# eduardburlacu/DiTSep

Measured on AMD Instinct MI355X. Metric: separated utterances/sec @ N=30, 2-spk 4 s mixtures, higher is better.
Workload: dtype fp16 (fp16 MFMA operands, fp32 accumulate)

## Files before the change

ditsep_amd/csrc/engine.hip:

```cpp
#include <math.h>
#include <stdarg.h>
#include <stdio.h>
#include <stdlib.h>
#include <string.h>

#include <algorithm>
#include <map>
#include <numeric>
#include <set>
#include <stdexcept>
#include <string>
#include <vector>

#include "../../include/ditsep_hip.h"
#include "igemm.h"
#include "kernels.h"

namespace {

struct Err : std::runtime_error {
  int code;
  Err(int c, const std::string& m) : std::runtime_error(m), code(c) {}
};

// ... 955 lines not shown
    op16_t* lnout = fp8 ? reinterpret_cast<op16_t*>(A8) : Ap;
    const char* skx = getenv("DSN_SKINNY_MAX");
    const int skinny_max = skx ? std::min(atoi(skx), 128) : 80;
    const bool skinny = P == 1 && !fp8 && M <= skinny_max && D % 256 == 0;
    const int skinny_ks = 8;
    const bool use_panel = D % 64 == 0;
    int fold_rows = 0;
    if ((fold_ln || fold_ln8) && use_panel && !skinny) {
      for (int rounds = 1; rounds <= 4 && !fold_rows; ++rounds) {
        const int np = 256 * rounds / std::max(1, cdiv(D, 128));
        if (np >= 1 && cdiv(M, np) <= 80) fold_rows = cdiv(M, np);
      }
    }
    op16_t* Xp = (fold_rows && !fp8) ? wsbuf<op16_t>("dit_Xp", M * D) : nullptr;
    unsigned char* X8 = (fold_rows && fp8) ? wsbuf<unsigned char>("dit_X8", M * D) : nullptr;
    unsigned char* SX8 = (fold_rows && fp8) ? wsbuf<unsigned char>("dit_SX8", M * D / 32) : nullptr;
    float* ST = fold_rows ? wsbuf<float>("dit_ST", M * (D / 64) * 2) : nullptr;
    const int rot = 32;
    const bool new_rope = !ws.count("rope_cos_" + std::to_string(S));
    float* rc = wsbuf<float>("rope_cos_" + std::to_string(S), (long)S * rot);
    float* rs = wsbuf<float>("rope_sin_" + std::to_string(S), (long)S * rot);
    if (new_rope) launch_rope_tables(rc, rs, S, rot, st);

    launch_pack_tokens(xt, io, mix, Dl, B, T, nullptr, Up, Mt * din, PL, st);
    {
      Tag tg(this, "dit.project_in");
      GemmDesc d = base_desc(Up, Mt * din, pin, B, T, T);
      d.out_f32 = X;
      d.out_bstride = (long)S * D;
      d.out_off = D;
      d.out_limit = (long)S * D;
      run(d, st);
    }
    {
      const float* te = time_cache.find(t, B);
      if (!te) {
        float* tmp = wsbuf<float>("dit_te1", (long)B * D);
        Tag tg(this, "dit.time_embed");
        dit_time_embed(t, B, tmp, st);
        te = tmp;
      }
      launch_copy_rows(te, X, B, D, (long)S * D, st);
    }
    const bool short_panel = use_panel && P == 1;
    auto panel_rows_for = [&](int wg_per_panel, int max_rows = 272) {
      for (int rounds = 1;; ++rounds) {
        const int np = std::max(1, 256 * rounds / std::max(1, wg_per_panel));
        const int rows = (cdiv(M, np) + 7) / 8 * 8;
        if (rows <= max_rows) return rows;
      }
    };
    const int qkv_panel = short_panel ? 256 : 0;
    int qa_ipp = 0;
    if (P == 1 && !skinny && D == H * 64 && S <= qkv_attention_max_rows()) {
      int ipp = std::min(B, std::max(1, 144 / S));
      while (ipp > 1 && cdiv(B, ipp) * H < 256) --ipp;
      if (cdiv(B, ipp) * H >= 128) qa_ipp = ipp;
      const char* force = getenv("DSN_QA_IPP");
      if (force && atoi(force) >= 1 && atoi(force) * S <= qkv_attention_max_rows()) qa_ipp = atoi(force);
    }
    op16_t* AOp = qa_ipp ? wsbuf<op16_t>("dit_AOp", M * D) : nullptr;
    float* slabs = nullptr;
    int pend_n = 0;
    const float* pend_bias = nullptr;
    const long slab_stride = M * D;
// ... 111 lines not shown
          d.out_fp8 = H8;
          d.out_fp8_scale = SH8;
        } else {
          d.out_planes = FF;
        }
        d.out_ps = M * 4 * D;
        d.out_bstride = M * 4L * D;
        d.out_row_elems = 4 * D;
        d.out_limit = d.out_bstride;
        d.m_fast = 1;
        if (use_panel) {
          const int np = cdiv(M, 272);
          d.panel_rows = short_panel ? panel_rows_for(cdiv(4 * D * 2, 256)) : (cdiv(M, np) + 7) / 8 * 8;
        }
        if (fp8) d.panel_rows = panel_rows_for(cdiv(4 * D * 2, 256));
        layer_gemm(d, 256, use_panel);
      }
      {
        Tag tg(this, "dit.ff_out");
        GemmDesc d = layer_desc(FF, H8, SH8, L.ff2, L.ff2_8);
        stream_gemm(d, 256, 4, fp8 ? 208 : 272);
      }
    }
    prof_launch("dit.residual_norm", (double)M * D * (8.0 + 4.0 * pend_n + 2.0 * P), st, [&] {
      launch_residual_norm(X, slabs, pend_n, slab_stride, pend_bias, nullptr, nullptr, Ap, M * D, PL, (int)M, D, 1e-5f,
                           0, st);
    });
    {
      Tag tg(this, "dit.project_out");
      GemmDesc d = base_desc(Ap, M * D, pout, B, T, S);
      d.in_pad = -1;
      d.in_bstride = (long)S * D;
      d.out_f32 = SC;
      if (use_panel && P == 1 && d.N <= 128 && d.M >= 1024) {
        d.panel_rows = 64;
        run(d, st, 128);
      } else {
        run(d, st);
      }
    }
    return SC;
  }

#include "engine_ncsnpp.inc"

  float* score_tokens(const float* xt, const float* t, const float* mix, int B, int T, hipStream_t st,
                      const int* lens = nullptr) {
    if (!finalized) fail(DSN_ESTATE, "weights not finalized");
    if (cfg.score_kind == DSN_SCORE_DIT) return dit_forward(xt, t, mix, B, T, st, lens);
    if (lens) fail(DSN_EINVAL, "ragged batches need the DiT score network");
    if (cfg.score_kind == DSN_SCORE_NCSNPP) {
      Tag tg(this, "ncsnpp.conv");
      return ncsnpp_forward(xt, t, mix, B, T, st);
    }
    fail(DSN_ESTATE, "no score network configured (score_kind=%d)", cfg.score_kind);
  }

  struct Sched {
    std::vector<float> t, std, step, gain, G, g;
// ... 1823 lines not shown
        q.M = (int)M;
        q.D = t->D;
        q.H = t->H;
        q.S = t->S;
        q.ipp = t->ipp;
        q.q_scale = 0.125f;
        const hipError_t e = qkv_attention_launch(q, PL, st, lens);
        if (e != hipSuccess)
          fail(DSN_EHIP, "test_kernel qkv_attention: refused or failed: %s (D=%d H=%d S=%d ipp=%d planes=%d)",
               hipGetErrorString(e), t->D, t->H, t->S, t->ipp, P);
        break;
      }
      case DSN_TK_RESIDUAL_NORM: {
        if (!t->x || t->rows < 1 || t->D < 4 || t->D % 4 != 0 || t->D > 4096)
          fail(DSN_EINVAL, "test_kernel residual_norm: needs x, rows >= 1, D %% 4 == 0, D <= 4096 (D=%d)", t->D);
        if (t->nslab < 0 || t->nslab > 8 || (t->nslab > 0 && !t->slabs))
          fail(DSN_EINVAL, "test_kernel residual_norm: nslab %d outside [0, 8] or slabs missing", t->nslab);
        if (t->do_norm && !t->gamma) fail(DSN_EINVAL, "test_kernel residual_norm: do_norm needs gamma");
        if (!!t->out_fp8 != !!t->out_fp8_scale || (!t->out_fp8 && !oplanes))
          fail(DSN_EINVAL, "test_kernel residual_norm: needs out_planes, or out_fp8 with out_fp8_scale");
        if (t->out_fp8 && t->D % 32 != 0) fail(DSN_EINVAL, "test_kernel residual_norm: fp8 output needs D %% 32 == 0");
        launch_residual_norm(t->x, t->slabs, t->nslab, t->slab_stride, t->bias, t->gamma, t->beta,
                             t->out_fp8 ? reinterpret_cast<op16_t*>(t->out_fp8) : oplanes, t->out_ps, PL, t->rows, t->D,
                             t->eps, t->do_norm, st, t->out_fp8_scale);
        break;
      }
      case DSN_TK_GN_STATS:
      case DSN_TK_GN_APPLY: {
        if (!t->x || t->B < 1 || t->HW < 1 || t->C % 4 != 0 || !gn_groups_fit(t->C, t->C) || t->C > 1024 ||
            t->rstride < t->C || t->rstride % 4 != 0)
          fail(DSN_EINVAL, "test_kernel group norm: unsupported view (C=%d rstride=%d HW=%d)", t->C, t->rstride, t->HW);
        if (t->kind == DSN_TK_GN_STATS) {
          if (!t->out_f32) fail(DSN_EINVAL, "test_kernel gn_stats: out_f32 (the statistics) missing");
          launch_gn_stats(t->x, t->bstride, t->rstride, t->C, t->B, t->HW, t->out_f32, st);
        } else {
          if (!t->stats || !t->gamma || !t->beta || (!t->out_f32 && !oplanes))
            fail(DSN_EINVAL, "test_kernel gn_apply: stats, gamma, beta and an output are required");
          launch_gn_apply(t->x, t->bstride, t->rstride, t->C, t->B, t->HW, t->stats, t->gamma, t->beta, t->eps, t->silu,
                          t->out_f32, oplanes, t->out_ps, PL, st);
        }
        break;
      }
      case DSN_TK_FIR2D: {
        if (!t->x || t->B < 1 || t->C < 4 || t->C % 4 != 0 || t->rstride < t->C || t->rstride % 4 != 0 || t->img_h < 1 ||
            t->img_w < 1 || (!t->up && ((t->img_h | t->img_w) & 1)) || (!t->out_f32 && !oplanes))
          fail(DSN_EINVAL, "test_kernel fir2d: unsupported view (C=%d rstride=%d %d x %d up=%d)", t->C, t->rstride,
               t->img_h, t->img_w, t->up);
// ... 215 lines not shown
```

ditsep_amd/csrc/igemm.hip:

```cpp
#include "igemm.h"

#ifndef DSN_SETPRIO
#define DSN_SETPRIO 0
#endif

namespace {

constexpr int BM = 128, BN = 128, BK = 32;
constexpr int TILE_ELEMS = 128 * BK;

__device__ __forceinline__ int swz(int row, int chunk) { return chunk ^ ((-(row >> 2)) & 3); }

enum { EPI_STATS = 1, EPI_LNFOLD = 2, EPI_FP8OUT = 4 };
enum { LEAN_NO_DIT = 1, LEAN_NO_NCSN = 2, LEAN_SEEDED = 4 };

template <int NT, int MT>
__device__ __forceinline__ void seed_acc(const GemmDesc& d, f32x4 (&acc)[NT][MT], int mw0, int m_end, int nw0, int lane) {
  const int nq = (lane >> 4) * 4;
#pragma unroll
  for (int tm = 0; tm < MT; ++tm) {
    const int m = mw0 + tm * 16 + (lane & 15);
    const bool mok = m < m_end;
    const int b = mok ? m / d.rows_per_b : 0;
    const int j = mok ? m - b * d.rows_per_b : 0;
// ... 1839 lines not shown
  if (d.panel_wm == 2 && d.cfg_bk == 32 && d.Cin % 32 != 0) return hipErrorInvalidValue;
  if (d.swiglu && (d.N % 32 != 0)) return hipErrorInvalidValue;
  if (d.ksplit > 1 && (!d.out_f32 || d.swiglu)) return hipErrorInvalidValue;
  if (d.img_w > 0) return hipErrorInvalidValue;
  if (d.stat_out && (d.N % 64 != 0 || d.stat_np != d.N / 64 || d.swiglu || d.ksplit > 1)) return hipErrorInvalidValue;
  if (d.ln_stats && (!d.swiglu || !d.ln_colsum || d.ln_np <= 0 || d.taps != 1 || planes != 1)) return hipErrorInvalidValue;
  const op16_t* zp = dsn_zero_page();
  if (!zp) return hipErrorOutOfMemory;
  const int epi = (d.stat_out ? EPI_STATS : 0) | (d.ln_stats ? EPI_LNFOLD : 0);
#define PCFGE(MT_, P_, W_, NS_, BK_, E_)                                                             \
  if (planes == P_ && bn == W_ * 64 && epi == E_)                                                     \
    return f16 ? launch_panel_t<P_, 1, W_, NS_, BK_, MT_, E_>(d, zp, stream)                          \
               : launch_panel_t<P_, 0, W_, NS_, BK_, MT_, E_>(d, zp, stream);
#define PCFGS(MT_, P_, W_, NS_, BK_) PCFGE(MT_, P_, W_, NS_, BK_, 0)
#define PCFG2(MT_, NS_, BK_, E_)                                                                                \
  if (planes == 1 && bn == 256 && epi == E_ && d.panel_rows <= MT_ * 16 && (d.cfg_nst == 0 || d.cfg_nst == NS_) && \
      (d.cfg_bk == 0 || d.cfg_bk == BK_))                                                                       \
    return f16 ? launch_panel_t<1, 1, 4, NS_, BK_, MT_, E_, 2>(d, zp, stream)                                   \
               : launch_panel_t<1, 0, 4, NS_, BK_, MT_, E_, 2>(d, zp, stream);
  if (d.panel_wm == 2) {
    PCFG2(9, 3, 64, 0) PCFG2(17, 2, 64, 0) PCFG2(17, 4, 32, 0) PCFG2(17, 2, 64, EPI_LNFOLD) PCFG2(17, 4, 32, EPI_LNFOLD)
  }
#undef PCFG2
  if (d.panel_rows <= 5 * 16) {
    PCFGE(5, 1, 2, 4, 64, EPI_STATS) PCFGS(5, 1, 2, 4, 64)
  }
  if (d.panel_rows <= 7 * 16) {
    PCFGS(7, 1, 4, 3, 64) PCFGE(7, 1, 4, 3, 64, EPI_LNFOLD)
  }
  if (d.panel_rows <= 9 * 16) {
    PCFGS(9, 1, 4, 3, 64) PCFGS(9, 1, 2, 3, 64) PCFGS(9, 2, 4, 2, 32) PCFGS(9, 2, 2, 2, 32)
    PCFGE(9, 1, 4, 3, 64, EPI_LNFOLD)
  }
  if (d.panel_rows <= 13 * 16) {
    PCFGS(13, 1, 4, 2, 64) PCFGS(13, 1, 2, 2, 64) PCFGE(13, 1, 4, 2, 64, EPI_LNFOLD)
  }
  PCFGS(17, 1, 4, 2, 64) PCFGS(17, 1, 2, 2, 64) PCFGS(17, 2, 4, 2, 32) PCFGS(17, 2, 2, 2, 32)
  PCFGE(17, 1, 4, 2, 64, EPI_LNFOLD)
#undef PCFGS
#undef PCFGE
  return hipErrorInvalidValue;
}
```

ditsep_amd/csrc/kernels.h:

```cpp
#pragma once
#include "common.h"

void launch_pack_tokens(const float* src0, int C0, const float* src1, int C1, int B, int T,
                        float* dst_f32, op16_t* dst_planes, long ps, int planes, hipStream_t s);
void launch_copy_rows(const float* src, float* dst, int rows, int width, long dst_stride, hipStream_t s);
void launch_unpack_tokens(const float* src, float* dst, int B, int C, int T, hipStream_t s);
void launch_to_planes(const float* src, op16_t* dst, long ps, int planes, long n, hipStream_t s);

void launch_pc_prior(const float* mean, int mean_full, const float* z, float* x, float stdT, int B, int n, int D,
                     int T, hipStream_t s);
void launch_pc_corrector(float* x, float* x_mean , const float* score_tok, const float* z, float step,
                         float noise_gain, const float* norms, float snr, int B, int n, int D, int T, hipStream_t s);
void launch_pc_item_norms(const float* a, long per_item, int B, float* out, hipStream_t s);
void launch_pc_predictor(float* x, float* x_mean, const float* y, const float* score_tok, const float* z,
                         float theta, float dt, float G, float g, int em, int B, int n, int D, int T, hipStream_t s);

void launch_sigma_mix(const float* y, float* smix, int B, int L, int avg_len, hipStream_t s);
void launch_mix_prior(const float* y, const float* z, float* x, const float* smix, float s1, float s2, int B, int n, int D,
                      int T, hipStream_t s);
void launch_mix_corrector(float* x, float* x_mean, const float* score_tok, const float* z, const float* smix, float sq1,
                          float sq2, float snr, int B, int n, int D, int T, hipStream_t s);
void launch_mix_predictor(float* x, float* x_mean, const float* score_tok, const float* z, const float* smix,
                          float lambda, float dt, float g, float sqdt, int em, int B, int n, int D, int T, hipStream_t s);
void launch_sb_update(float* x, const float* est_tok, const float* third, float w_prev, float w_est, float w3,
                      int third_is_y, int B, int n, int D, int T, hipStream_t s);
void launch_repeat_sources(const float* y, float* x, int B, int n, int D, int T, hipStream_t s);
void launch_zero_tail(float* x, const int* lens, int B, int n, int D, int T, hipStream_t s);

void launch_residual_norm(float* x, const float* slabs, int nslab, long slab_stride, const float* bias,
                          const float* gamma, const float* beta, op16_t* out, long ps, int planes, int rows, int D,
                          float eps, int do_norm, hipStream_t s, unsigned char* out_fp8_scale = nullptr);
void launch_timestep_features(const float* t, const float* w, int B, int half, op16_t* out, long ps,
                              int planes, hipStream_t s);
hipError_t launch_attention_mfma(const op16_t* qkv, long ps, op16_t* out, long out_ps, int pl, int B, int S, int H,
                                 int dh, hipStream_t s, unsigned char* out_fp8_scale = nullptr,
                                 const int* lens = nullptr);
void launch_rope_tables(float* cos_t, float* sin_t, int S, int rot, hipStream_t s);

void launch_conv_out1(const op16_t* a, long ps, int planes, const float* w, float* out, int S, int L, int C,
                      int ktaps, int apply_tanh, hipStream_t s);
void launch_conv_in1(const float* wav, const float* w, const float* bias, int S, int L, int Cout, int ktaps,
                     float* out_f32, op16_t* out_planes, long ps, int planes, int act, const float* act_a,
                     const float* act_b, hipStream_t s);
void launch_vae_sample(const float* enc_tok, const float* noise, float* y, int S, int D, int T, hipStream_t s);

void launch_randn(float* out, long n, unsigned long long seed, unsigned long long offset, hipStream_t s);

enum { PACK_LINEAR = 0, PACK_LINEAR_SWIGLU = 1, PACK_CONV = 2, PACK_CONVT = 3, PACK_CONV2D = 4, PACK_NIN = 5 };
void launch_wn_scale(const float* v, const float* g, float* scale, int R, long inner, hipStream_t s);
void launch_pack_weight(const float* src, const float* scale, op16_t* dst, long ps, int planes, int mode,
                        int N, int K, int Cin, int Cout, int kw, int stride, hipStream_t s,
                        const float* colscale = nullptr);
void launch_packed_row_sum(const op16_t* w, long ps, int planes, int N, int K, float* out, hipStream_t s);
void launch_bias_plus_wbeta(const float* W, const float* beta, const float* bias, int N, int K, float* out,
// ... 121 lines not shown
```

ditsep_amd/csrc/kernels.hip:

```cpp
#include "kernels.h"

namespace {

constexpr int TPB = 256;
inline int grid_for(long n, int per_block = TPB, int cap = 256 * 16) {
  long g = (n + per_block - 1) / per_block;
  return (int)(g < 1 ? 1 : (g > cap ? cap : g));
}

__device__ __forceinline__ void store_planes(op16_t* dst, long ps, int planes, long i, float v) {
  op16_t h, l;
  dsn_split(v, h, l, PL_F16(planes));
  dst[i] = h;
  if (PL_COUNT(planes) == 2) dst[ps + i] = l;
}

__global__ void pack_tokens_kernel(const float* __restrict__ s0, int C0, const float* __restrict__ s1, int C1,
                                   int B, int T, float* __restrict__ df, op16_t* __restrict__ dp, long ps,
                                   int planes) {
  const int C = C0 + C1;
  const long n = (long)B * T * C;
  for (long i = blockIdx.x * (long)blockDim.x + threadIdx.x; i < n; i += (long)gridDim.x * blockDim.x) {
    const int c = (int)(i % C);
    const long bt = i / C;
    const int t = (int)(bt % T);
    const int b = (int)(bt / T);
    const float v = c < C0 ? s0[((long)b * C0 + c) * T + t] : s1[((long)b * C1 + (c - C0)) * T + t];
    if (df) df[i] = v;
    if (dp) store_planes(dp, ps, planes, i, v);
  }
}

__global__ void copy_rows_kernel(const float* __restrict__ src, float* __restrict__ dst, int rows, int width4,
                                 long dst_stride) {
  const long n = (long)rows * width4;
  for (long i = blockIdx.x * (long)blockDim.x + threadIdx.x; i < n; i += (long)gridDim.x * blockDim.x) {
    const long r = i / width4;
    const int c = (int)(i - r * width4);
    reinterpret_cast<f32x4*>(dst + r * dst_stride)[c] = reinterpret_cast<const f32x4*>(src + r * (long)width4 * 4)[c];
  }
}

__global__ void unpack_tokens_kernel(const float* __restrict__ src, float* __restrict__ dst, int B, int C, int T) {
  const long n = (long)B * C * T;
  for (long i = blockIdx.x * (long)blockDim.x + threadIdx.x; i < n; i += (long)gridDim.x * blockDim.x) {
    const int t = (int)(i % T);
    const long bc = i / T;
    const int c = (int)(bc % C);
    const int b = (int)(bc / C);
    dst[i] = src[((long)b * T + t) * C + c];
  }
}

__global__ void to_planes_kernel(const float* __restrict__ src, op16_t* __restrict__ dst, long ps, int planes,
                                 long n4) {
  for (long i = blockIdx.x * (long)blockDim.x + threadIdx.x; i < n4; i += (long)gridDim.x * blockDim.x) {
    const f32x4 v = reinterpret_cast<const f32x4*>(src)[i];
    op16x4 hi, lo;
#pragma unroll
    for (int r = 0; r < 4; ++r) {
      op16_t h, l;
      dsn_split(v[r], h, l, PL_F16(planes));
// ... 199 lines not shown
    const float th = third ? third[third_is_y ? ix.yi : i] : 0.f;
    x[i] = w_prev * x[i] + w_est * est[ix.si] + w3 * th;
  }
}
__global__ void repeat_sources_kernel(const float* __restrict__ y, float* __restrict__ x, int n, int D, int T, long total) {
  for (long i = blockIdx.x * (long)blockDim.x + threadIdx.x; i < total; i += (long)gridDim.x * blockDim.x)
    x[i] = y[pc_index(i, n, D, T).yi];
}

__global__ void zero_tail_kernel(float* __restrict__ x, const int* __restrict__ lens, int rows, int T, long total) {
  for (long i = blockIdx.x * (long)blockDim.x + threadIdx.x; i < total; i += (long)gridDim.x * blockDim.x) {
    const int t = (int)(i % T);
    const int b = (int)(i / ((long)rows * T));
    if (t >= lens[b] - 1) x[i] = 0.f;
  }
}

template <int MAXV, int NS, bool BATCH = false>
__global__ __launch_bounds__(TPB) void residual_norm_kernel(float* __restrict__ x, const float* __restrict__ slabs,
                                                            int nslab, long slab_stride, const float* __restrict__ bias,
                                                            const float* __restrict__ gamma,
                                                            const float* __restrict__ beta, op16_t* __restrict__ out,
                                                            long ps, int planes, int rows, int D, float eps, int do_norm,
                                                            unsigned char* __restrict__ o8s) {
  const int lane = threadIdx.x & 63;
  const int wpb = blockDim.x >> 6;
  const int nv = D >> 2;
  for (int row = blockIdx.x * wpb + (threadIdx.x >> 6); row < rows; row += gridDim.x * wpb) {
    const long rbase = (long)row * D;
    f32x4 v[MAXV];
    f32x4 gq[BATCH ? MAXV : 1], bq[BATCH ? MAXV : 1];
    float s = 0.f;
    if constexpr (BATCH) {
      f32x4 bv[MAXV];
      f32x4 part[NS > 0 ? NS : 1][MAXV];
#pragma unroll
      for (int k = 0; k < MAXV; ++k) {
        const int i = min(lane + k * 64, nv - 1);
        v[k] = reinterpret_cast<const f32x4*>(x + rbase)[i];
        bv[k] = (NS > 0 && bias) ? reinterpret_cast<const f32x4*>(bias)[i] : f32x4{0.f, 0.f, 0.f, 0.f};
#pragma unroll
        for (int z = 0; z < NS; ++z) part[z][k] = reinterpret_cast<const f32x4*>(slabs + z * slab_stride + rbase)[i];
      }
#pragma unroll
      for (int k = 0; k < MAXV; ++k) {
        const int i = lane + k * 64;
        if (do_norm) {
          gq[k] = reinterpret_cast<const f32x4*>(gamma)[min(i, nv - 1)];
          bq[k] = beta ? reinterpret_cast<const f32x4*>(beta)[min(i, nv - 1)] : f32x4{0.f, 0.f, 0.f, 0.f};
        }
        v[k] += bv[k];
#pragma unroll
        for (int z = 0; z < NS; ++z) v[k] += part[z][k];
        if (i < nv) {
          if (NS > 0) reinterpret_cast<f32x4*>(x + rbase)[i] = v[k];
          s += (v[k][0] + v[k][1]) + (v[k][2] + v[k][3]);
        }
      }
    } else {
#pragma unroll
      for (int k = 0; k < MAXV; ++k) {
        const int i = lane + k * 64;
        if (i < nv) {
          f32x4 a = reinterpret_cast<const f32x4*>(x + rbase)[i];
          if (NS > 0) {
            f32x4 part[NS > 0 ? NS : 1];
#pragma unroll
            for (int z = 0; z < NS; ++z) part[z] = reinterpret_cast<const f32x4*>(slabs + z * slab_stride + rbase)[i];
            if (bias) a += reinterpret_cast<const f32x4*>(bias)[i];
#pragma unroll
            for (int z = 0; z < NS; ++z) a += part[z];
            reinterpret_cast<f32x4*>(x + rbase)[i] = a;
          }
          v[k] = a;
          s += (a[0] + a[1]) + (a[2] + a[3]);
        }
      }
    }
    float mean = 0.f, rstd = 1.f;
    if (do_norm) {
      mean = wave_sum(s) / D;
      float q = 0.f;
#pragma unroll
      for (int k = 0; k < MAXV; ++k) {
        const int i = lane + k * 64;
        if (i < nv) {
#pragma unroll
          for (int r = 0; r < 4; ++r) {
            const float dlt = v[k][r] - mean;
            q += dlt * dlt;
          }
        }
      }
      rstd = rsqrtf(wave_sum(q) / D + eps);
    }
// ... 25 lines not shown
        }
        op16x4 hi, lo;
#pragma unroll
        for (int r = 0; r < 4; ++r) {
          op16_t h, l;
          dsn_split(o[r], h, l, PL_F16(planes));
          hi[r] = h;
          lo[r] = l;
        }
        const long oi = (rbase >> 2) + i;
        reinterpret_cast<op16x4*>(out)[oi] = hi;
        if (PL_COUNT(planes) == 2) reinterpret_cast<op16x4*>(out + ps)[oi] = lo;
      }
    }
  }
}

template <int NS>
__global__ __launch_bounds__(TPB) void residual_norm_row_kernel(float* __restrict__ x, const float* __restrict__ slabs,
                                                                long slab_stride, const float* __restrict__ bias,
                                                                const float* __restrict__ gamma,
                                                                const float* __restrict__ beta, op16_t* __restrict__ out,
                                                                long ps, int planes, int D, float eps, int do_norm,
                                                                unsigned char* __restrict__ o8s) {
  __shared__ float red[2][TPB / 64];
  const int i = threadIdx.x, lane = i & 63, wave = i >> 6;
  const long rbase = (long)blockIdx.x * D;
  f32x4 a = reinterpret_cast<const f32x4*>(x + rbase)[i];
  f32x4 part[NS > 0 ? NS : 1];
#pragma unroll
  for (int z = 0; z < NS; ++z) part[z] = reinterpret_cast<const f32x4*>(slabs + z * slab_stride + rbase)[i];
  f32x4 g = {1.f, 1.f, 1.f, 1.f}, be = {0.f, 0.f, 0.f, 0.f};
  if (do_norm) {
    g = reinterpret_cast<const f32x4*>(gamma)[i];
    if (beta) be = reinterpret_cast<const f32x4*>(beta)[i];
  }
  if (NS > 0) {
    if (bias) a += reinterpret_cast<const f32x4*>(bias)[i];
#pragma unroll
    for (int z = 0; z < NS; ++z) a += part[z];
    reinterpret_cast<f32x4*>(x + rbase)[i] = a;
  }
  f32x4 o = a;
  if (do_norm) {
    const float s = wave_sum((a[0] + a[1]) + (a[2] + a[3]));
    if (lane == 0) red[0][wave] = s;
    __syncthreads();
    float tot = 0.f;
#pragma unroll
    for (int w = 0; w < TPB / 64; ++w) tot += red[0][w];
    const float mean = tot / D;
    float q = 0.f;
#pragma unroll
    for (int r = 0; r < 4; ++r) {
      const float dlt = a[r] - mean;
      q += dlt * dlt;
    }
    q = wave_sum(q);
    if (lane == 0) red[1][wave] = q;
    __syncthreads();
    float qt = 0.f;
#pragma unroll
    for (int w = 0; w < TPB / 64; ++w) qt += red[1][w];
    const float rstd = rsqrtf(qt / D + eps);
// ... 436 lines not shown
  s = wave_sum(s);
  if (lane == 0) out[row] = s + (bias ? bias[row] : 0.f);
}

__global__ void pack_bias_swiglu_kernel(const float* __restrict__ src, float* __restrict__ dst, int N) {
  const int F = N / 2;
  for (int n = blockIdx.x * blockDim.x + threadIdx.x; n < N; n += gridDim.x * blockDim.x) {
    const int g = n >> 5, w = n & 31;
    dst[n] = src[w < 16 ? 16 * g + w : F + 16 * g + (w - 16)];
  }
}

__global__ void snake_params_kernel(const float* __restrict__ alpha, const float* __restrict__ beta,
                                    float* __restrict__ a, float* __restrict__ ib, int C) {
  for (int i = blockIdx.x * blockDim.x + threadIdx.x; i < C; i += gridDim.x * blockDim.x) {
    a[i] = expf(alpha[i]);
    ib[i] = 1.0f / (expf(beta[i]) + 1e-9f);
  }
}

}

void launch_pack_tokens(const float* s0, int C0, const float* s1, int C1, int B, int T, float* df, op16_t* dp,
                        long ps, int planes, hipStream_t st) {
  const long n = (long)B * T * (C0 + C1);
  hipLaunchKernelGGL(pack_tokens_kernel, dim3(grid_for(n)), dim3(TPB), 0, st, s0, C0, s1, C1, B, T, df, dp, ps,
                     planes);
}
void launch_copy_rows(const float* src, float* dst, int rows, int width, long dst_stride, hipStream_t st) {
  hipLaunchKernelGGL(copy_rows_kernel, dim3(grid_for((long)rows * (width / 4))), dim3(TPB), 0, st, src, dst, rows,
                     width / 4, dst_stride);
}
void launch_unpack_tokens(const float* src, float* dst, int B, int C, int T, hipStream_t st) {
  hipLaunchKernelGGL(unpack_tokens_kernel, dim3(grid_for((long)B * C * T)), dim3(TPB), 0, st, src, dst, B, C, T);
}
void launch_to_planes(const float* src, op16_t* dst, long ps, int planes, long n, hipStream_t st) {
  hipLaunchKernelGGL(to_planes_kernel, dim3(grid_for(n / 4)), dim3(TPB), 0, st, src, dst, ps, planes, n / 4);
}
void launch_pc_prior(const float* mean, int mean_full, const float* z, float* x, float stdT, int B, int n, int D,
                     int T, hipStream_t st) {
  const long total = (long)B * n * D * T;
  hipLaunchKernelGGL(pc_prior_kernel, dim3(grid_for(total)), dim3(TPB), 0, st, mean, z, x, stdT, n, D, T, total,
                     mean_full);
}
void launch_pc_corrector(float* x, float* xm, const float* sc, const float* z, float step, float gain,
                         const float* norms, float snr, int B, int n, int D, int T, hipStream_t st) {
  const long total = (long)B * n * D * T;
  hipLaunchKernelGGL(pc_corrector_kernel, dim3(grid_for(total)), dim3(TPB), 0, st, x, xm, sc, z, step, gain, norms,
                     B, snr, n, D, T, total);
}
void launch_pc_item_norms(const float* a, long per_item, int B, float* out, hipStream_t st) {
  hipLaunchKernelGGL(pc_item_norm_kernel, dim3(B), dim3(256), 0, st, a, per_item, out);
}
void launch_pc_predictor(float* x, float* xm, const float* y, const float* sc, const float* z, float theta,
// ... 19 lines not shown
}
void launch_mix_predictor(float* x, float* xm, const float* sc, const float* z, const float* smix, float lambda, float dt,
                          float g, float sqdt, int em, int B, int n, int D, int T, hipStream_t st) {
  const long npos = (long)B * D * T;
  hipLaunchKernelGGL(mix_predictor_kernel, dim3(grid_for(npos)), dim3(TPB), 0, st, x, xm, sc, z, smix, lambda, dt, g,
                     sqdt, em, n, D, T, npos);
}
void launch_sb_update(float* x, const float* est, const float* third, float w_prev, float w_est, float w3, int third_is_y,
                      int B, int n, int D, int T, hipStream_t st) {
  const long total = (long)B * n * D * T;
  hipLaunchKernelGGL(sb_update_kernel, dim3(grid_for(total)), dim3(TPB), 0, st, x, est, third, w_prev, w_est, w3,
                     third_is_y, n, D, T, total);
}
void launch_repeat_sources(const float* y, float* x, int B, int n, int D, int T, hipStream_t st) {
  const long total = (long)B * n * D * T;
  hipLaunchKernelGGL(repeat_sources_kernel, dim3(grid_for(total)), dim3(TPB), 0, st, y, x, n, D, T, total);
}
void launch_zero_tail(float* x, const int* lens, int B, int n, int D, int T, hipStream_t st) {
  const long total = (long)B * n * D * T;
  hipLaunchKernelGGL(zero_tail_kernel, dim3(grid_for(total)), dim3(TPB), 0, st, x, lens, n * D, T, total);
}
void launch_residual_norm(float* x, const float* slabs, int nslab, long slab_stride, const float* bias,
                          const float* gamma, const float* beta, op16_t* out, long ps, int planes, int rows, int D,
                          float eps, int do_norm, hipStream_t st, unsigned char* o8s) {
#define RN_LAUNCH(MV, NS_, BT_)                                                                                       \
  hipLaunchKernelGGL((residual_norm_kernel<MV, NS_, BT_>), dim3(grid_for(rows, 4)), dim3(TPB), 0, st, x, slabs, nslab, \
                     slab_stride, bias, gamma, beta, out, ps, planes, rows, D, eps, do_norm, o8s)
#define RN_SWITCH(MV, BT_)                                                                 \
  switch (nslab) {                                                                         \
    case 0: RN_LAUNCH(MV, 0, BT_); break;                                                  \
    case 1: RN_LAUNCH(MV, 1, BT_); break;                                                  \
    case 2: RN_LAUNCH(MV, 2, BT_); break;                                                  \
    case 3: RN_LAUNCH(MV, 3, BT_); break;                                                  \
    case 4: RN_LAUNCH(MV, 4, BT_); break;                                                  \
    case 5: RN_LAUNCH(MV, 5, BT_); break;                                                  \
    case 6: RN_LAUNCH(MV, 6, BT_); break;                                                  \
    case 7: RN_LAUNCH(MV, 7, BT_); break;                                                  \
    default: RN_LAUNCH(MV, 8, BT_); break;            \
  }
  if (D == 4 * TPB && rows > 256 && nslab <= 4) {
#define RNR(NS_)                                                                                                     \
  hipLaunchKernelGGL((residual_norm_row_kernel<NS_>), dim3(rows), dim3(TPB), 0, st, x, slabs, slab_stride, bias, gamma, \
                     beta, out, ps, planes, D, eps, do_norm, o8s)
    switch (nslab) {
      case 0: RNR(0); break;
      case 1: RNR(1); break;
      case 2: RNR(2); break;
      case 3: RNR(3); break;
      default: RNR(4); break;
    }
#undef RNR
    return;
  }
  if (D <= 1024 && rows <= 256) {
    RN_SWITCH(4, true)
  } else if (D <= 1024) {
    RN_SWITCH(4, false)
  } else {
    RN_SWITCH(16, false)
  }
#undef RN_SWITCH
#undef RN_LAUNCH
}
void launch_timestep_features(const float* t, const float* w, int B, int half, op16_t* out, long ps, int planes,
                              hipStream_t st) {
  hipLaunchKernelGGL(timestep_features_kernel, dim3(grid_for((long)B * half)), dim3(TPB), 0, st, t, w, B, half,
// ... 115 lines not shown
```

ditsep_amd/native.py:

```python
from __future__ import annotations

import ctypes as C
import math
import os
import warnings
from typing import Mapping, Optional

import torch

_HERE = os.path.dirname(os.path.abspath(__file__))
LIB_PATH = os.environ.get("DSN_LIB", os.path.join(_HERE, "libditsep_hip.so"))

PREC_BF16 = 1
PREC_BF16X3 = 2
PREC_FP16 = 3
PREC_FP16X3 = 4
PREC_FP8 = 5
SCORE_NONE, SCORE_DIT, SCORE_NCSNPP = 0, 1, 2
MAX_VAE_BLOCKS = 8

EXPORTS = [
    "dsn_create", "dsn_destroy", "dsn_last_error", "dsn_load_tensor", "dsn_finalize_weights", "dsn_finalize_weights_ex",
    "dsn_score", "dsn_score_ragged", "dsn_pc_sample_ragged", "dsn_ouve_schedule", "dsn_pc_sample", "dsn_pc_sample_sched", "dsn_pc_sample_ex", "dsn_pc_sample_mix", "dsn_sb_sample", "dsn_decode",
    "dsn_encode", "dsn_decode_chunked", "dsn_encode_chunked",
# ... 94 lines not shown
        ("panel_rows", C.c_int), ("panel_bn", C.c_int), ("panel_wm", C.c_int), ("ksplit", C.c_int),
        ("B", C.c_int), ("Lin", C.c_int), ("Cin", C.c_int), ("N", C.c_int), ("taps", C.c_int), ("in_stride", C.c_int),
        ("tap_dil", C.c_int), ("in_pad", C.c_int), ("rows_per_b", C.c_int), ("M", C.c_int),
        ("in_row_elems", C.c_int), ("a_off", C.c_int), ("in_bstride", C.c_int64),
        ("img_h", C.c_int), ("img_w", C.c_int), ("out_bstride", C.c_int64),
        ("out_row_elems", C.c_int), ("out_off", C.c_int), ("out_limit", C.c_int64),
        ("a", C.c_void_p), ("a_numel", C.c_int64), ("w", C.c_void_p),
        ("bias", C.c_void_p), ("bias_mod", C.c_int), ("bbias", C.c_void_p), ("bbias_stride", C.c_int),
        ("resid", C.c_void_p), ("resid_bstride", C.c_int64), ("resid_row_elems", C.c_int), ("resid_off", C.c_int),
        ("out_scale", C.c_float), ("f32_op", C.c_int), ("act", C.c_int), ("act_a", C.c_void_p), ("act_b", C.c_void_p),
        ("act_mod", C.c_int), ("swiglu", C.c_int), ("gn_stats", C.c_void_p), ("gn_stats2", C.c_void_p),
        ("gn_nq2", C.c_int), ("gn_qoff2", C.c_int),
        ("sc_a", C.c_void_p), ("sc_a_numel", C.c_int64), ("sc_w", C.c_void_p), ("sc_bias", C.c_void_p),
        ("sc_Cin", C.c_int), ("sc_row_elems", C.c_int),
        ("out_f32", C.c_void_p), ("out_planes", C.c_void_p), ("out_ps", C.c_int64),
        ("slabs", C.c_void_p), ("slab_stride", C.c_int64),
    ]


TEST_KERNEL_KINDS = {"attention": 1, "qkv_attention": 2, "residual_norm": 3, "gn_stats": 4, "gn_apply": 5, "fir2d": 6,
                     "conv_out1": 7, "conv_in1": 8, "ru_fused": 9,
                     "pc_prior": 10, "pc_corrector": 11, "pc_item_norms": 12, "pc_predictor": 13, "sigma_mix": 14,
                     "mix_prior": 15, "mix_corrector": 16, "mix_predictor": 17, "sb_update": 18, "repeat_sources": 19,
                     "vae_sample": 20, "randn": 21, "rand_uniform": 22}


class DsnTestKernel(C.Structure):
    _fields_ = [
        ("kind", C.c_int), ("B", C.c_int), ("S", C.c_int), ("H", C.c_int), ("dh", C.c_int), ("D", C.c_int),
        ("ipp", C.c_int), ("rows", C.c_int), ("nslab", C.c_int), ("do_norm", C.c_int), ("eps", C.c_float),
        ("slab_stride", C.c_int64),
        ("C", C.c_int), ("HW", C.c_int), ("rstride", C.c_int), ("img_h", C.c_int), ("img_w", C.c_int), ("up", C.c_int),
        ("silu", C.c_int), ("bstride", C.c_int64),
        ("L", C.c_int), ("ktaps", C.c_int), ("apply_tanh", C.c_int), ("act", C.c_int),
        ("dil", C.c_int), ("act_out", C.c_int),
        ("a", C.c_void_p), ("a_numel", C.c_int64), ("w", C.c_void_p), ("w_numel", C.c_int64), ("w2", C.c_void_p),
        ("w2_numel", C.c_int64), ("x", C.c_void_p),
        ("slabs", C.c_void_p), ("bias", C.c_void_p), ("bias2", C.c_void_p), ("gamma", C.c_void_p), ("beta", C.c_void_p),
        ("stats", C.c_void_p), ("add", C.c_void_p), ("act_a", C.c_void_p), ("act_b", C.c_void_p),
        ("out_act_a", C.c_void_p), ("out_act_b", C.c_void_p), ("rope_cos", C.c_void_p), ("rope_sin", C.c_void_p),
        ("out_f32", C.c_void_p), ("out_planes", C.c_void_p), ("out_ps", C.c_int64), ("out_fp8", C.c_void_p),
        ("out_fp8_scale", C.c_void_p),
        ("n", C.c_int), ("T", C.c_int), ("avg_len", C.c_int), ("em", C.c_int), ("mean_full", C.c_int),
        ("third_is_y", C.c_int),
        ("stdT", C.c_float), ("step", C.c_float), ("gain", C.c_float), ("snr", C.c_float), ("theta", C.c_float),
        ("dt", C.c_float), ("G", C.c_float), ("g", C.c_float), ("s1", C.c_float), ("s2", C.c_float), ("lam", C.c_float),
        ("sqdt", C.c_float), ("w_prev", C.c_float), ("w_est", C.c_float), ("w3", C.c_float), ("lo", C.c_float),
        ("hi", C.c_float),
        ("seed", C.c_uint64), ("offset", C.c_uint64), ("count", C.c_int64),
        ("y", C.c_void_p), ("score", C.c_void_p), ("z", C.c_void_p), ("smix", C.c_void_p), ("norms", C.c_void_p),
        ("xmean", C.c_void_p),
        ("lens", C.c_void_p),
    ]


def latent_frames_of(L: int, hop: int) -> int:
    return int(L) // int(hop) + 1


def ragged_extended_length(L: int, hop: int) -> int:
    return latent_frames_of(L, hop) * int(hop) - 1


def frame_groups(frames) -> dict:
    groups: dict = {}
    for i, f in enumerate(frames):
        groups.setdefault(int(f), []).append(i)
    return groups


def check_ragged(score_kind: int, frames, B: int, T: int, corrector: str = "ald") -> list:
    if score_kind != SCORE_DIT:
        raise ValueError("ragged batches need the DiT score network: NCSN++ convolves across time, so padding would "
                         "change an item's result")
    fr = [int(f) for f in frames]
# ... 677 lines not shown
```

include/ditsep_hip.h:

```cpp
#ifndef DITSEP_HIP_H
#define DITSEP_HIP_H

#include <stdint.h>

#ifdef __cplusplus
extern "C" {
#endif

#define DSN_OK 0
#define DSN_EINVAL (-1)
#define DSN_EHIP (-2)
#define DSN_ESTATE (-3)
#define DSN_ENOMEM (-4)
#define DSN_ESOLVER (-5)

#define DSN_PREC_BF16 1
#define DSN_PREC_BF16X3 2
#define DSN_PREC_FP16 3
#define DSN_PREC_FP16X3 4
#define DSN_PREC_FP8 5

#define DSN_SCORE_NONE 0
#define DSN_SCORE_DIT 1
#define DSN_SCORE_NCSNPP 2
// ... 198 lines not shown
  int act_mod;
  int swiglu;
  float* gn_stats;
  float* gn_stats2;
  int gn_nq2, gn_qoff2;
  const float* sc_a;
  int64_t sc_a_numel;
  const float* sc_w;
  const float* sc_bias;
  int sc_Cin, sc_row_elems;
  float* out_f32;
  int16_t* out_planes;
  int64_t out_ps;
  float* slabs;
  int64_t slab_stride;
} DsnTestGemm;
int dsn_test_gemm(dsn_ctx* ctx, const DsnTestGemm* t, void* stream);

enum { DSN_TK_ATTENTION = 1, DSN_TK_QKV_ATTENTION = 2, DSN_TK_RESIDUAL_NORM = 3, DSN_TK_GN_STATS = 4,
       DSN_TK_GN_APPLY = 5, DSN_TK_FIR2D = 6, DSN_TK_CONV_OUT1 = 7, DSN_TK_CONV_IN1 = 8, DSN_TK_RU_FUSED = 9,
       DSN_TK_PC_PRIOR = 10, DSN_TK_PC_CORRECTOR = 11, DSN_TK_PC_ITEM_NORMS = 12, DSN_TK_PC_PREDICTOR = 13,
       DSN_TK_SIGMA_MIX = 14, DSN_TK_MIX_PRIOR = 15, DSN_TK_MIX_CORRECTOR = 16, DSN_TK_MIX_PREDICTOR = 17,
       DSN_TK_SB_UPDATE = 18, DSN_TK_REPEAT_SOURCES = 19, DSN_TK_VAE_SAMPLE = 20, DSN_TK_RANDN = 21,
       DSN_TK_RAND_UNIFORM = 22 };
typedef struct DsnTestKernel {
  int kind;
  int B, S, H, dh, D, ipp;
  int rows, nslab, do_norm;
  float eps;
  int64_t slab_stride;
  int C, HW, rstride, img_h, img_w, up, silu;
  int64_t bstride;
  int L, ktaps, apply_tanh, act;
  int dil, act_out;
  const float* a;
  int64_t a_numel;
  const float* w;
  int64_t w_numel;
  const float* w2;
  int64_t w2_numel;
  float* x;
  const float* slabs;
  const float* bias;
  const float* bias2;
  const float* gamma;
  const float* beta;
  const float* stats;
  const float* add;
  const float* act_a;
  const float* act_b;
  const float* out_act_a;
  const float* out_act_b;
  float* rope_cos;
  float* rope_sin;
  float* out_f32;
  int16_t* out_planes;
  int64_t out_ps;
  uint8_t* out_fp8;
  uint8_t* out_fp8_scale;
  int n, T, avg_len, em, mean_full, third_is_y;
  float stdT, step, gain, snr, theta, dt, G, g, s1, s2, lam, sqdt, w_prev, w_est, w3, lo, hi;
  uint64_t seed, offset;
  int64_t count;
  const float* y;
  const float* score;
  const float* z;
  const float* smix;
  const float* norms;
  float* xmean;
  const int32_t* lens;
} DsnTestKernel;
int dsn_test_kernel(dsn_ctx* ctx, const DsnTestKernel* t, void* stream);

int dsn_debug_read(dsn_ctx* ctx, const char* name, float* host, int64_t count);
int dsn_bench_igemm(dsn_ctx* ctx, int B, int Lin, int Cin, int N, int taps, int tap_dil, int in_pad, int ksplit,
                    int variant, int iters, double* ms_out);

#ifdef __cplusplus
}
#endif
#endif
```

Before: 288.5.

## Fuse time-embed row copy into token packing, skip final residual store, narrow panels

```diff
diff --git a/ditsep_amd/csrc/engine.hip b/ditsep_amd/csrc/engine.hip
--- a/ditsep_amd/csrc/engine.hip
+++ b/ditsep_amd/csrc/engine.hip
@@ -1001,7 +1001,16 @@
     float* rs = wsbuf<float>("rope_sin_" + std::to_string(S), (long)S * rot);
     if (new_rope) launch_rope_tables(rc, rs, S, rot, st);
 
-    launch_pack_tokens(xt, io, mix, Dl, B, T, nullptr, Up, Mt * din, PL, st);
+    {
+      const float* te = time_cache.find(t, B);
+      if (!te) {
+        float* tmp = wsbuf<float>("dit_te1", (long)B * D);
+        Tag tg(this, "dit.time_embed");
+        dit_time_embed(t, B, tmp, st);
+        te = tmp;
+      }
+      launch_pack_tokens(xt, io, mix, Dl, B, T, nullptr, Up, Mt * din, PL, st, te, X, D, (long)S * D);
+    }
     {
       Tag tg(this, "dit.project_in");
       GemmDesc d = base_desc(Up, Mt * din, pin, B, T, T);
@@ -1009,17 +1018,13 @@
       d.out_bstride = (long)S * D;
       d.out_off = D;
       d.out_limit = (long)S * D;
-      run(d, st);
-    }
-    {
-      const float* te = time_cache.find(t, B);
-      if (!te) {
-        float* tmp = wsbuf<float>("dit_te1", (long)B * D);
-        Tag tg(this, "dit.time_embed");
-        dit_time_embed(t, B, tmp, st);
-        te = tmp;
-      }
-      launch_copy_rows(te, X, B, D, (long)S * D, st);
+      if (use_panel && P == 1 && d.Cin % 64 == 0 && d.M >= 1024) {
+        d.panel_rows = 32;
+        d.panel_wm = 1;
+        run(d, st, 128);
+      } else {
+        run(d, st);
+      }
     }
     const bool short_panel = use_panel && P == 1;
     auto panel_rows_for = [&](int wg_per_panel, int max_rows = 272) {
@@ -1177,9 +1182,9 @@
         stream_gemm(d, 256, 4, fp8 ? 208 : 272);
       }
     }
-    prof_launch("dit.residual_norm", (double)M * D * (8.0 + 4.0 * pend_n + 2.0 * P), st, [&] {
+    prof_launch("dit.residual_norm", (double)M * D * (4.0 + 4.0 * pend_n + 2.0 * P), st, [&] {
       launch_residual_norm(X, slabs, pend_n, slab_stride, pend_bias, nullptr, nullptr, Ap, M * D, PL, (int)M, D, 1e-5f,
-                           0, st);
+                           0, st, nullptr, 0);
     });
     {
       Tag tg(this, "dit.project_out");
@@ -1188,8 +1193,9 @@
       d.in_bstride = (long)S * D;
       d.out_f32 = SC;
       if (use_panel && P == 1 && d.N <= 128 && d.M >= 1024) {
-        d.panel_rows = 64;
-        run(d, st, 128);
+        d.panel_rows = 32;
+        d.panel_wm = 1;
+        run(d, st, 64);
       } else {
         run(d, st);
       }
@@ -3059,7 +3065,16 @@
         if (t->out_fp8 && t->D % 32 != 0) fail(DSN_EINVAL, "test_kernel residual_norm: fp8 output needs D %% 32 == 0");
         launch_residual_norm(t->x, t->slabs, t->nslab, t->slab_stride, t->bias, t->gamma, t->beta,
                              t->out_fp8 ? reinterpret_cast<op16_t*>(t->out_fp8) : oplanes, t->out_ps, PL, t->rows, t->D,
-                             t->eps, t->do_norm, st, t->out_fp8_scale);
+                             t->eps, t->do_norm, st, t->out_fp8_scale, !t->skip_x_store);
+        break;
+      }
+      case DSN_TK_PACK_TOKENS: {
+        if (!t->x || !t->out_f32 || t->B < 1 || t->T < 1 || t->C < 1)
+          fail(DSN_EINVAL, "test_kernel pack_tokens: needs x [B][C][T], out_f32 [B*T][C], B, T, C");
+        if (t->add && (!t->xmean || t->D < 4 || t->D % 4 != 0 || t->bstride < t->D || t->bstride % 4 != 0))
+          fail(DSN_EINVAL, "test_kernel pack_tokens: placed rows need xmean, D %% 4 == 0, bstride >= D, bstride %% 4 == 0");
+        launch_pack_tokens(t->x, t->C, nullptr, 0, t->B, t->T, t->out_f32, nullptr, 0, PL, st, t->add, t->xmean, t->D,
+                           t->bstride);
         break;
       }
       case DSN_TK_GN_STATS:
diff --git a/ditsep_amd/csrc/igemm.hip b/ditsep_amd/csrc/igemm.hip
--- a/ditsep_amd/csrc/igemm.hip
+++ b/ditsep_amd/csrc/igemm.hip
@@ -1885,6 +1885,15 @@
     PCFG2(9, 3, 64, 0) PCFG2(17, 2, 64, 0) PCFG2(17, 4, 32, 0) PCFG2(17, 2, 64, EPI_LNFOLD) PCFG2(17, 4, 32, EPI_LNFOLD)
   }
 #undef PCFG2
+#define PCFG1(W_)                                                                                \
+  if (planes == 1 && bn == W_ * 64 && epi == 0 && d.panel_rows <= 32)                             \
+    return f16 ? launch_panel_t<1, 1, W_, 4, 64, 2, 0, 2>(d, zp, stream)                          \
+               : launch_panel_t<1, 0, W_, 4, 64, 2, 0, 2>(d, zp, stream);
+  if (d.panel_wm == 1) {
+    PCFG1(2) PCFG1(1)
+    return hipErrorInvalidValue;
+  }
+#undef PCFG1
   if (d.panel_rows <= 5 * 16) {
     PCFGE(5, 1, 2, 4, 64, EPI_STATS) PCFGS(5, 1, 2, 4, 64)
   }
diff --git a/ditsep_amd/csrc/kernels.h b/ditsep_amd/csrc/kernels.h
--- a/ditsep_amd/csrc/kernels.h
+++ b/ditsep_amd/csrc/kernels.h
@@ -2,8 +2,8 @@
 #include "common.h"
 
 void launch_pack_tokens(const float* src0, int C0, const float* src1, int C1, int B, int T,
-                        float* dst_f32, op16_t* dst_planes, long ps, int planes, hipStream_t s);
-void launch_copy_rows(const float* src, float* dst, int rows, int width, long dst_stride, hipStream_t s);
+                        float* dst_f32, op16_t* dst_planes, long ps, int planes, hipStream_t s,
+                        const float* te = nullptr, float* xrows = nullptr, int width = 0, long xstride = 0);
 void launch_unpack_tokens(const float* src, float* dst, int B, int C, int T, hipStream_t s);
 void launch_to_planes(const float* src, op16_t* dst, long ps, int planes, long n, hipStream_t s);
 
@@ -29,7 +29,8 @@
 
 void launch_residual_norm(float* x, const float* slabs, int nslab, long slab_stride, const float* bias,
                           const float* gamma, const float* beta, op16_t* out, long ps, int planes, int rows, int D,
-                          float eps, int do_norm, hipStream_t s, unsigned char* out_fp8_scale = nullptr);
+                          float eps, int do_norm, hipStream_t s, unsigned char* out_fp8_scale = nullptr,
+                          int store_x = 1);
 void launch_timestep_features(const float* t, const float* w, int B, int half, op16_t* out, long ps,
                               int planes, hipStream_t s);
 hipError_t launch_attention_mfma(const op16_t* qkv, long ps, op16_t* out, long out_ps, int pl, int B, int S, int H,
diff --git a/ditsep_amd/csrc/kernels.hip b/ditsep_amd/csrc/kernels.hip
--- a/ditsep_amd/csrc/kernels.hip
+++ b/ditsep_amd/csrc/kernels.hip
@@ -17,7 +17,8 @@
 
 __global__ void pack_tokens_kernel(const float* __restrict__ s0, int C0, const float* __restrict__ s1, int C1,
                                    int B, int T, float* __restrict__ df, op16_t* __restrict__ dp, long ps,
-                                   int planes) {
+                                   int planes, const float* __restrict__ te, float* __restrict__ xrows, int width4,
+                                   long xstride) {
   const int C = C0 + C1;
   const long n = (long)B * T * C;
   for (long i = blockIdx.x * (long)blockDim.x + threadIdx.x; i < n; i += (long)gridDim.x * blockDim.x) {
@@ -29,15 +30,13 @@
     if (df) df[i] = v;
     if (dp) store_planes(dp, ps, planes, i, v);
   }
-}
-
-__global__ void copy_rows_kernel(const float* __restrict__ src, float* __restrict__ dst, int rows, int width4,
-                                 long dst_stride) {
-  const long n = (long)rows * width4;
-  for (long i = blockIdx.x * (long)blockDim.x + threadIdx.x; i < n; i += (long)gridDim.x * blockDim.x) {
-    const long r = i / width4;
-    const int c = (int)(i - r * width4);
-    reinterpret_cast<f32x4*>(dst + r * dst_stride)[c] = reinterpret_cast<const f32x4*>(src + r * (long)width4 * 4)[c];
+  if (te) {
+    const long nq = (long)B * width4;
+    for (long i = blockIdx.x * (long)blockDim.x + threadIdx.x; i < nq; i += (long)gridDim.x * blockDim.x) {
+      const long r = i / width4;
+      const int c = (int)(i - r * width4);
+      reinterpret_cast<f32x4*>(xrows + r * xstride)[c] = reinterpret_cast<const f32x4*>(te + r * (long)width4 * 4)[c];
+    }
   }
 }
 
@@ -283,7 +282,7 @@
                                                             const float* __restrict__ gamma,
                                                             const float* __restrict__ beta, op16_t* __restrict__ out,
                                                             long ps, int planes, int rows, int D, float eps, int do_norm,
-                                                            unsigned char* __restrict__ o8s) {
+                                                            int store_x, unsigned char* __restrict__ o8s) {
   const int lane = threadIdx.x & 63;
   const int wpb = blockDim.x >> 6;
   const int nv = D >> 2;
@@ -314,7 +313,7 @@
 #pragma unroll
         for (int z = 0; z < NS; ++z) v[k] += part[z][k];
         if (i < nv) {
-          if (NS > 0) reinterpret_cast<f32x4*>(x + rbase)[i] = v[k];
+          if (NS > 0 && store_x) reinterpret_cast<f32x4*>(x + rbase)[i] = v[k];
           s += (v[k][0] + v[k][1]) + (v[k][2] + v[k][3]);
         }
       }
@@ -331,7 +330,7 @@
             if (bias) a += reinterpret_cast<const f32x4*>(bias)[i];
 #pragma unroll
             for (int z = 0; z < NS; ++z) a += part[z];
-            reinterpret_cast<f32x4*>(x + rbase)[i] = a;
+            if (store_x) reinterpret_cast<f32x4*>(x + rbase)[i] = a;
           }
           v[k] = a;
           s += (a[0] + a[1]) + (a[2] + a[3]);
@@ -403,7 +402,7 @@
                                                                 const float* __restrict__ gamma,
                                                                 const float* __restrict__ beta, op16_t* __restrict__ out,
                                                                 long ps, int planes, int D, float eps, int do_norm,
-                                                                unsigned char* __restrict__ o8s) {
+                                                                int store_x, unsigned char* __restrict__ o8s) {
   __shared__ float red[2][TPB / 64];
   const int i = threadIdx.x, lane = i & 63, wave = i >> 6;
   const long rbase = (long)blockIdx.x * D;
@@ -420,7 +419,7 @@
     if (bias) a += reinterpret_cast<const f32x4*>(bias)[i];
 #pragma unroll
     for (int z = 0; z < NS; ++z) a += part[z];
-    reinterpret_cast<f32x4*>(x + rbase)[i] = a;
+    if (store_x) reinterpret_cast<f32x4*>(x + rbase)[i] = a;
   }
   f32x4 o = a;
   if (do_norm) {
@@ -903,14 +902,10 @@
 }
 
 void launch_pack_tokens(const float* s0, int C0, const float* s1, int C1, int B, int T, float* df, op16_t* dp,
-                        long ps, int planes, hipStream_t st) {
+                        long ps, int planes, hipStream_t st, const float* te, float* xrows, int width, long xstride) {
   const long n = (long)B * T * (C0 + C1);
   hipLaunchKernelGGL(pack_tokens_kernel, dim3(grid_for(n)), dim3(TPB), 0, st, s0, C0, s1, C1, B, T, df, dp, ps,
-                     planes);
-}
-void launch_copy_rows(const float* src, float* dst, int rows, int width, long dst_stride, hipStream_t st) {
-  hipLaunchKernelGGL(copy_rows_kernel, dim3(grid_for((long)rows * (width / 4))), dim3(TPB), 0, st, src, dst, rows,
-                     width / 4, dst_stride);
+                     planes, te, xrows, width / 4, xstride);
 }
 void launch_unpack_tokens(const float* src, float* dst, int B, int C, int T, hipStream_t st) {
   hipLaunchKernelGGL(unpack_tokens_kernel, dim3(grid_for((long)B * C * T)), dim3(TPB), 0, st, src, dst, B, C, T);
@@ -976,10 +971,10 @@
 }
 void launch_residual_norm(float* x, const float* slabs, int nslab, long slab_stride, const float* bias,
                           const float* gamma, const float* beta, op16_t* out, long ps, int planes, int rows, int D,
-                          float eps, int do_norm, hipStream_t st, unsigned char* o8s) {
+                          float eps, int do_norm, hipStream_t st, unsigned char* o8s, int store_x) {
 #define RN_LAUNCH(MV, NS_, BT_)                                                                                       \
   hipLaunchKernelGGL((residual_norm_kernel<MV, NS_, BT_>), dim3(grid_for(rows, 4)), dim3(TPB), 0, st, x, slabs, nslab, \
-                     slab_stride, bias, gamma, beta, out, ps, planes, rows, D, eps, do_norm, o8s)
+                     slab_stride, bias, gamma, beta, out, ps, planes, rows, D, eps, do_norm, store_x, o8s)
 #define RN_SWITCH(MV, BT_)                                                                 \
   switch (nslab) {                                                                         \
     case 0: RN_LAUNCH(MV, 0, BT_); break;                                                  \
@@ -995,7 +990,7 @@
   if (D == 4 * TPB && rows > 256 && nslab <= 4) {
 #define RNR(NS_)                                                                                                     \
   hipLaunchKernelGGL((residual_norm_row_kernel<NS_>), dim3(rows), dim3(TPB), 0, st, x, slabs, slab_stride, bias, gamma, \
-                     beta, out, ps, planes, D, eps, do_norm, o8s)
+                     beta, out, ps, planes, D, eps, do_norm, store_x, o8s)
     switch (nslab) {
       case 0: RNR(0); break;
       case 1: RNR(1); break;
diff --git a/ditsep_amd/native.py b/ditsep_amd/native.py
--- a/ditsep_amd/native.py
+++ b/ditsep_amd/native.py
@@ -140,7 +140,7 @@
                      "conv_out1": 7, "conv_in1": 8, "ru_fused": 9,
                      "pc_prior": 10, "pc_corrector": 11, "pc_item_norms": 12, "pc_predictor": 13, "sigma_mix": 14,
                      "mix_prior": 15, "mix_corrector": 16, "mix_predictor": 17, "sb_update": 18, "repeat_sources": 19,
-                     "vae_sample": 20, "randn": 21, "rand_uniform": 22}
+                     "vae_sample": 20, "randn": 21, "rand_uniform": 22, "pack_tokens": 23}
 
 
 class DsnTestKernel(C.Structure):
@@ -169,6 +169,7 @@
         ("y", C.c_void_p), ("score", C.c_void_p), ("z", C.c_void_p), ("smix", C.c_void_p), ("norms", C.c_void_p),
         ("xmean", C.c_void_p),
         ("lens", C.c_void_p),
+        ("skip_x_store", C.c_int),
     ]
 
 
diff --git a/include/ditsep_hip.h b/include/ditsep_hip.h
--- a/include/ditsep_hip.h
+++ b/include/ditsep_hip.h
@@ -244,7 +244,7 @@
        DSN_TK_PC_PRIOR = 10, DSN_TK_PC_CORRECTOR = 11, DSN_TK_PC_ITEM_NORMS = 12, DSN_TK_PC_PREDICTOR = 13,
        DSN_TK_SIGMA_MIX = 14, DSN_TK_MIX_PRIOR = 15, DSN_TK_MIX_CORRECTOR = 16, DSN_TK_MIX_PREDICTOR = 17,
        DSN_TK_SB_UPDATE = 18, DSN_TK_REPEAT_SOURCES = 19, DSN_TK_VAE_SAMPLE = 20, DSN_TK_RANDN = 21,
-       DSN_TK_RAND_UNIFORM = 22 };
+       DSN_TK_RAND_UNIFORM = 22, DSN_TK_PACK_TOKENS = 23 };
 typedef struct DsnTestKernel {
   int kind;
   int B, S, H, dh, D, ipp;
@@ -291,6 +291,7 @@
   const float* norms;
   float* xmean;
   const int32_t* lens;
+  int skip_x_store;
 } DsnTestKernel;
 int dsn_test_kernel(dsn_ctx* ctx, const DsnTestKernel* t, void* stream);
 
```

Result: no change. 290.0, median of 6 (+0.5%).
